# latentnetworks/vimure

Measured on AMD Instinct MI355X. Metric: CAVI iterations/sec (L=4 N=2000 M=200 K=2 synthetic, mutuality on), higher is better.
Workload: dtype f64

## Files before the change

vimure_amd/csrc/sweep_sl.h:

```cpp
#ifndef VMR_SWEEP_SL_H
#define VMR_SWEEP_SL_H

#include "vmr_internal.h"
#include <functional>

#define SL_YM(e) ((e) & 0xfffffu)
#define SL_INR(e) (((e) >> 20) & 1u)
#define SL_X(e) ((e) >> 21)
#define SL_XMAX 2047u
#define SL_YM_ROWS (1u << 20)
#define SL_PF 8
#ifndef SL_PFW
#define SL_PFW 8
#endif
constexpr int sl_pf(int K) { return K <= 2 ? SL_PF : SL_PFW; }
#define SL_SLACK (64 * 64)

struct SlArgs {
  const unsigned* E; const unsigned* rs; const unsigned long long* ebase; const unsigned* perm;
  const unsigned* sy;
  const uint8_t* cls;
  const unsigned* Qt;
  const uint64_t* Rb; const unsigned* rq; const unsigned short* Rm; const unsigned long long* rbase;
  const unsigned* rm2;
  double* rho; const double* logpr;
  const double* par; double* slotR; const double* lutg; double* Hg; double* slotF; double* slotA;
  int Gl;
  int do_hist;
  int yt, hc;
  int sum_a;
  double* nu_acc; double* elbo_dev; int commit_nu;
  int nu_stale;
  unsigned long long* det;
  int lp0;
  int farl;
  double* h0s;
  const unsigned* x0p;
  int lv0r;
  const unsigned* Ez;
  int elbo_cur;
#ifdef SL_DEBUG
  unsigned long long* dbg_t;
#endif
};

struct SlShape { int tpb, yt, hc; size_t smem; };
struct SlUnit { SlArgs a; Geo g; int blk0, nblk; };

#ifndef SL_LIGHT_UPD_K
#define SL_LIGHT_UPD_K 2
#endif
constexpr bool sl_light(int K, bool elbo, bool allfull, bool update) { return !elbo && allfull && (K <= SL_LIGHT_UPD_K || (!update && K <= 4)); }
#ifndef SL_ELBO3_K
#define SL_ELBO3_K 2
#endif
#ifndef SL_ELBO3
#define SL_ELBO3 1
#endif
constexpr int sl_tpb_max(int K, bool elbo, bool allfull, bool update = true) {
  return elbo ? ((SL_ELBO3 && K <= SL_ELBO3_K) ? 768 : (K <= 4 ? 512 : 256)) : (sl_light(K, elbo, allfull, update) ? 1024 : (K <= 3 ? 768 : (K <= 7 ? 512 : 256)));
}
constexpr int sl_tpb_max_b(int K, bool elbo, bool allfull) { return elbo ? sl_tpb_max(K, true, allfull) : (K <= 2 ? 768 : (K <= 7 ? 512 : 256)); }
constexpr int sl_wpe_b(int K, bool elbo, bool allfull) { return elbo ? ((SL_ELBO3 && K <= SL_ELBO3_K) ? 3 : (K <= 4 ? 2 : 1)) : (K <= 2 ? 3 : (K <= 7 ? 2 : 1)); }
// ... 24 lines not shown
```

vimure_amd/csrc/sweep_sl.hip:

```cpp
#include "sweep_sl.h"

#ifndef VMR_K
#error "compile with -DVMR_K=<number of categories>"
#endif
#ifndef SL_WPE
#define SL_WPE sl_wpe(2, false, true)
#endif

template <int K>
struct StepIn {
  double v[K];
  double w[K];
  unsigned cls, qt, tie;
  unsigned x0;
  unsigned e[sl_pf(K)];
};

template <int R> struct RC { static constexpr int value = R; };
template <class V> __device__ __forceinline__ const V* at_bytes(const V* p, unsigned off) {
  return reinterpret_cast<const V*>(reinterpret_cast<const char*>(p) + off);
}
template <class V> __device__ __forceinline__ V* at_bytes(V* p, unsigned off) {
  return reinterpret_cast<V*>(reinterpret_cast<char*>(p) + off);
}
__device__ __forceinline__ double rcp_nr2(double d) {
  double r = __builtin_amdgcn_rcp(d);
  r = fma(fma(-d, r, 1.0), r, r);
  return fma(fma(-d, r, 1.0), r, r);
}
#define SL_INL __attribute__((always_inline))
#ifndef SL_BATCH2
#define SL_BATCH2 8
#endif
template <int K> struct Batch { static constexpr int value = K <= 2 ? SL_BATCH2 : (K <= 4 ? 4 : 2); };

template <int K, bool UPDATE, bool ELBO, bool ALLFULL, bool STORE = true, bool DET = false>
__device__ __forceinline__ void sweep_body(const SlArgs& a, const Geo& g, const unsigned bx, const unsigned gx) {
  extern __shared__ __align__(16) unsigned char smem[];
  constexpr int PFK = sl_pf(K);
  constexpr bool LV0 = !UPDATE && !ELBO && !DET;
  constexpr bool LV0R = UPDATE && K >= 3;
  const int tid = threadIdx.x, lane = tid & 63, nthr = (int)blockDim.x;
  const int wv = __builtin_amdgcn_readfirstlane(tid >> 6), nw = nthr >> 6;
  const int Mp = g.Mp;
  const unsigned ytm = UPDATE ? (unsigned)a.yt * (unsigned)Mp : 0u;
  const unsigned hcm = a.do_hist ? (unsigned)a.hc * (unsigned)Mp : 0u;
  size_t off = 0;
  double* F = reinterpret_cast<double*>(smem + off); off += (size_t)ytm * K * 8;
  const int nHc = (int)hcm * K;
  double* Hc = reinterpret_cast<double*>(smem + off); off += (size_t)nHc * 8;
  double* Gth = reinterpret_cast<double*>(smem + off); off += (size_t)Mp * 8;
  double* Lth = reinterpret_cast<double*>(smem + off); off += UPDATE ? (size_t)Mp * 8 : 0;
  double* As = reinterpret_cast<double*>(smem + off); off += a.sum_a ? (size_t)Mp * K * 8 : 0;
  double* wsum = reinterpret_cast<double*>(smem + off); off += (size_t)g.W * 8;
  double* red = reinterpret_cast<double*>(smem + off); off += 16 * 8;
  double* xt = reinterpret_cast<double*>(smem + off); off += 64 * 8;
  double* lt = reinterpret_cast<double*>(smem + off); off += ELBO ? 256 * 8 : 0;
  double* EthL = reinterpret_cast<double*>(smem + off); off += a.rq ? (size_t)Mp * 8 : 0;
  const ParOff o = par_off(g.L, g.Mp, g.K);
// ... 39 lines not shown
  const double lp0_0 = log(1.0 + eps), lp0_k = log(eps);
  double e_lin = 0.0, e_q = 0.0, e_log = 0.0;
  double accF[K], acc0[K];
#pragma unroll
  for (int k = 0; k < K; ++k) { accF[k] = 0.0; acc0[k] = 0.0; }
  unsigned long long ie_lin = 0ull, ie_q = 0ull, ie_log = 0ull, iaccF[K];
#pragma unroll
  for (int k = 0; k < K; ++k) iaccF[k] = 0ull;
  double* Hl = a.Hg + ((size_t)l * NH + (gb % NH)) * g.Y * Mp * K;
  auto det_H = [&]() SL_INL { return a.det + (size_t)l * g.Y * Mp * K; };
  auto det_A = [&]() SL_INL { return a.det + (size_t)g.L * g.Y * Mp * K + (size_t)l * g.W * 64 * K; };
  auto det_F = [&]() SL_INL { return a.det + (size_t)g.L * g.Y * Mp * K + (size_t)g.L * g.W * 64 * K + (size_t)l * K; };
  auto det_R = [&]() SL_INL { return a.det + (size_t)g.L * g.Y * Mp * K + (size_t)g.L * g.W * 64 * K + (size_t)g.L * K; };
  const unsigned* rsl = a.rs + (size_t)l * (NS + 1);
  const unsigned* syl = a.sy + (size_t)l * NS;
  const unsigned* El = a.E + a.ebase[l];
  const unsigned* pl = (a.rm2 ? a.rm2 : a.perm) + (size_t)l * NS * 64;
  const uint8_t* cl = ALLFULL ? nullptr : a.cls + (size_t)l * T;
  const unsigned* Ql = a.Qt ? a.Qt + (size_t)l * T : nullptr;
  const uint64_t* Rl = a.Rb ? a.Rb + (size_t)l * T * g.W : nullptr;
  double* rl = a.rho + (size_t)l * T * K;
  double* rho_slack = a.rho + (size_t)g.L * T * K;
  const double* lpl = a.logpr + (size_t)l * T * K;
  const unsigned* rql = a.rq ? a.rq + (size_t)l * (T + 1) : nullptr;
  const unsigned short* Rml = a.rq ? a.Rm + a.rbase[l] : nullptr;
  const unsigned lim_y = UPDATE ? (a.do_hist ? (unsigned)min(a.yt, a.hc) : (unsigned)a.yt) : (a.do_hist ? (unsigned)a.hc : 0xffffffffu);
  const unsigned lim1 = (UPDATE && a.yt < g.Y) ? (unsigned)a.yt : 0xffffffffu;
  const unsigned lim2 = (a.do_hist && a.hc < g.Y) ? (unsigned)a.hc : 0xffffffffu;

  const long long Gl_ = a.Gl;
  unsigned* tick = reinterpret_cast<unsigned*>(smem + off); off += 16;
  if (tid == 0) { tick[0] = 2u * (unsigned)nw; tick[1] = 0u; }
  auto step_of = [&](unsigned t) SL_INL -> long long { return (long long)gb + (long long)t * Gl_; };
  auto draw = [&]() SL_INL -> long long {
    unsigned t = 0u;
    if (lane == 0) t = atomicAdd(tick, 1u);
    return step_of((unsigned)__builtin_amdgcn_readfirstlane((int)t));
  };
  long long s = step_of((unsigned)wv), sn = step_of((unsigned)(nw + wv));
  unsigned ea = 0;
  int R = 0;
  unsigned ymax = 0;
  unsigned rgv = 0;
  StepIn<K> P;

  const unsigned lane4 = (unsigned)lane * 4u, laneK8 = (unsigned)lane * (unsigned)(K * 8);
  const unsigned T32 = (unsigned)T;
  auto fetch_range = [&](long long st) SL_INL {
    const unsigned ra = rsl[st + (lane < 1 ? 0 : 1)], ry = syl[st];
    rgv = lane == 2 ? ry : ra;
  };
  auto fetch_tie = [&](StepIn<K>& d, long long st, const bool lp_const = false) SL_INL {
    const size_t row0 = (size_t)st * 64;
    const bool ok = (unsigned)row0 + (unsigned)lane < T32;
    d.qt = 0u; d.tie = 0u;
    if (ALLFULL) d.cls = ok ? 1u : 0u;
    else {
      const unsigned c = (unsigned)*at_bytes(cl + row0, (unsigned)lane);
      d.cls = ok ? c : 0u;
      d.tie = *at_bytes(pl + row0, lane4);
    }
    if (ELBO && Ql) d.qt = *at_bytes(Ql + row0, lane4);
    d.x0 = 0u;
    if (LV0 && a.x0p) d.x0 = *at_bytes(a.x0p + (size_t)l * NS * 64 + row0, lane4);
#pragma unroll
    for (int k = 0; k < K; ++k) { d.v[k] = 0.0; d.w[k] = 0.0; }
    if (UPDATE || ELBO) {
      if (lp_const) {
#pragma unroll
        for (int k = 0; k < K; ++k) d.v[k] = k == 0 ? lp0_0 : lp0_k;
      } else load_k<K>(at_bytes(lpl + row0 * K, laneK8), d.v);
    }
    if (!UPDATE && a.do_hist != 2) load_k<K>(at_bytes(static_cast<const double*>(rl) + row0 * K, laneK8), d.w);
  };
  auto fetch_ent = [&](StepIn<K>& d, unsigned base, auto cntc) SL_INL {
    constexpr int CNT = decltype(cntc)::value;
    const unsigned* pe = El + base;
#pragma unroll
    for (int j = 0; j < CNT; ++j) d.e[j] = *at_bytes(pe + j * 64, lane4);
  };

  if (s < NS) {
    ea = rsl[s];
    R = (int)((rsl[s + 1] - ea) >> 6);
    ymax = syl[s];
    fetch_range(sn < NS ? sn : s);
    fetch_tie(P, s);
    fetch_ent(P, ea, RC<PFK>{});
  }
#ifdef SL_DEBUG
// ... 232 lines not shown
            const double dx = fr[u] ? 0.0 : (double)SL_X(c[u]);
#pragma unroll
            for (int k = 0; k < K; ++k) U[k] = fma(dx, f[u][k], U[k]);
          }
#pragma unroll
          for (int u = 0; u < GB; ++u) {
            if (__any(fr[u])) {
              if (fr[u]) {
                double ff[K];
                f_far(SL_YM(c[u]), ff);
                const double dx = (double)SL_X(c[u]);
#pragma unroll
                for (int k = 0; k < K; ++k) U[k] = fma(dx, ff[k], U[k]);
              }
            }
          }
        }, Rr);
        if (LV0R && a.lv0r && !lv0_off) {
#pragma unroll
          for (int k = 0; k < K; ++k) U[k] += fma(Lla[k], sx1, sl0);
        }
      }
      double aa[K];
#pragma unroll
      for (int k = 0; k < K; ++k) aa[k] = (cur.v[k] + U[k]) - Tt * Ela[k];
      bool done = false;
      if (K == 2) {
        const double d = aa[1] - aa[0];
        const bool safe = fabs(aa[0]) < 700.0 && fabs(aa[1]) < 700.0 && fabs(d) < 700.0;
        if (__all(safe)) {
          const double e = exp_tab(d, xt);
          r[0] = rcp_nr2(1.0 + e);
          r[1] = e * r[0];
          done = true;
        }
      }
      if (!done) {
        double sum = 0.0;
        bool tame = true;
#pragma unroll
        for (int k = 0; k < K; ++k) tame = tame && fabs(aa[k]) < 700.0;
        tame = __all(tame);
        if (tame) {
#pragma unroll
          for (int k = 0; k < K; ++k) r[k] = exp_tab(aa[k], xt);
        } else {
#pragma unroll
          for (int k = 0; k < K; ++k) r[k] = exp(aa[k]);
        }
#pragma unroll
        for (int k = 0; k < K; ++k) sum += r[k];
        if (sum > 0.0) {
#pragma unroll
          for (int k = 0; k < K; ++k) r[k] /= sum;
        }
        if (a.do_hist) {
          double sm = 0.0;
#pragma unroll
// ... 302 lines not shown
    }
  }
  if (ELBO) {
    if (DET) {
      const unsigned long long v1 = wave_isum(ie_lin), v2 = wave_isum(ie_log), v3 = wave_isum(ie_q);
      if (lane == 0) { unsigned long long* dR = det_R(); atomicAdd(&dR[1], v1); atomicAdd(&dR[2], v2); atomicAdd(&dR[3], v3); }
    } else {
      double v1 = block_sum_n(e_lin, red);
      double v2 = block_sum_n(e_log, red);
      double v3 = block_sum_n(e_q, red);
      if (tid == 0) {
        double* out = a.slotR + (size_t)(bx % NSLOT) * 4;
        atomicAdd(&out[1], v1); atomicAdd(&out[2], v2); atomicAdd(&out[3], v3);
      }
    }
  }
#ifdef SL_DEBUG
  if (dbt && lane == 0) dbt[3] = wall_clock64();
#endif
}

#define SL_BOUNDS(K, UPDATE, ELBO, ALLFULL) \
  __launch_bounds__(sl_tpb_max(K, ELBO, ALLFULL, UPDATE), (K == 2 && !ELBO && ALLFULL) ? SL_WPE : sl_wpe(K, ELBO, ALLFULL, UPDATE))
template <int K, bool UPDATE, bool ELBO, bool ALLFULL, bool STORE = true, bool DET = false>
__global__ SL_BOUNDS(K, UPDATE, ELBO, ALLFULL) void k_sweep_sl(SlArgs a, Geo g) {
  sweep_body<K, UPDATE, ELBO, ALLFULL, STORE, DET>(a, g, blockIdx.x, gridDim.x);
}
template <int K, bool UPDATE, bool ELBO, bool ALLFULL, bool STORE = true>
__global__ __launch_bounds__(sl_tpb_max_b(K, ELBO, ALLFULL), sl_wpe_b(K, ELBO, ALLFULL)) void k_sweep_sl_b(const SlUnit* __restrict__ units, const int* __restrict__ blk_unit) {
  const SlUnit& u = units[blk_unit[blockIdx.x]];
  sweep_body<K, UPDATE, ELBO, ALLFULL, STORE>(u.a, u.g, blockIdx.x - (unsigned)u.blk0, (unsigned)u.nblk);
}

template <bool UPDATE, bool ELBO, bool ALLFULL, bool STORE = true, bool DET = false>
static int sl_launch_one(vmr_ctx* h, const SlShape& sh, SlArgs& a) {
  constexpr int K = VMR_K;
  const Geo& g = h->g;
  const long long NS = ((long long)g.N * g.N + 63) / 64, nw = sh.tpb / 64;
  int rc = grid_per_layer(h, k_sweep_sl<K, UPDATE, ELBO, ALLFULL, STORE, DET>, sh.smem, &a.Gl, (NS + nw - 1) / nw, sh.tpb);
  if (rc) return rc;
#ifdef SL_DEBUG
  static unsigned long long* dbg_buf = nullptr;
  const char* tf = h->opt.debug_times[0] ? h->opt.debug_times : nullptr;
  const size_t nwv = (size_t)g.L * a.Gl * nw;
  a.dbg_t = nullptr;
  if (tf) {
    if (!dbg_buf) (void)hipMalloc(&dbg_buf, (size_t)1 << 22);
    if (nwv * 64 <= ((size_t)1 << 22)) a.dbg_t = dbg_buf;
  }
#endif
  hipLaunchKernelGGL((k_sweep_sl<K, UPDATE, ELBO, ALLFULL, STORE, DET>), dim3(g.L * a.Gl), dim3(sh.tpb), sh.smem, h->stream, a, g);
#ifdef SL_DEBUG
  if (a.dbg_t) {
    std::vector<unsigned long long> t(nwv * 8);
    (void)hipStreamSynchronize(h->stream);
    (void)hipMemcpy(t.data(), dbg_buf, nwv * 64, hipMemcpyDeviceToHost);
    if (FILE* f = fopen(tf, "a")) {
      fprintf(f, "launch %d%d hist %d waves %zu tpb %d\n", (int)UPDATE, (int)ELBO, a.do_hist, nwv, sh.tpb);
      for (size_t i = 0; i < nwv; ++i) fprintf(f, "%llu %llu %llu %llu %llu %llu %llu %llu\n", t[i * 8], t[i * 8 + 1], t[i * 8 + 2], t[i * 8 + 3], t[i * 8 + 4], t[i * 8 + 5], t[i * 8 + 6], t[i * 8 + 7]);
      fclose(f);
    }
  }
#endif
  return VMR_OK;
}

#define SL_CAT2(a, b) a##b
#define SL_CAT(a, b) SL_CAT2(a, b)
int SL_CAT(vmr_sl_launch_k, VMR_K)(vmr_ctx* h, int mode, const SlShape& sh, SlArgs& a) {
  if (a.det) {
    if (a.cls == nullptr) {
      switch (mode) {
        case 0: return sl_launch_one<true, false, true, true, true>(h, sh, a);
        case 4: return sl_launch_one<true, false, true, false, true>(h, sh, a);
        case 1: return sl_launch_one<true, true, true, true, true>(h, sh, a);
        case 2: return sl_launch_one<false, true, true, true, true>(h, sh, a);
        default: return sl_launch_one<false, false, true, true, true>(h, sh, a);
      }
    }
    switch (mode) {
      case 0: return sl_launch_one<true, false, false, true, true>(h, sh, a);
      case 4: return sl_launch_one<true, false, false, false, true>(h, sh, a);
      case 1: return sl_launch_one<true, true, false, true, true>(h, sh, a);
      case 2: return sl_launch_one<false, true, false, true, true>(h, sh, a);
      default: return sl_launch_one<false, false, false, true, true>(h, sh, a);
    }
  }
  if (a.cls == nullptr) {
    switch (mode) {
      case 0: return sl_launch_one<true, false, true>(h, sh, a);
      case 1: return sl_launch_one<true, true, true>(h, sh, a);
      case 2: return sl_launch_one<false, true, true>(h, sh, a);
      case 4: return sl_launch_one<true, false, true, false>(h, sh, a);
      default: return sl_launch_one<false, false, true>(h, sh, a);
    }
  }
  switch (mode) {
    case 0: return sl_launch_one<true, false, false>(h, sh, a);
    case 1: return sl_launch_one<true, true, false>(h, sh, a);
    case 2: return sl_launch_one<false, true, false>(h, sh, a);
    case 4: return sl_launch_one<true, false, false, false>(h, sh, a);
    default: return sl_launch_one<false, false, false>(h, sh, a);
  }
}

template <bool UPDATE, bool ELBO, bool ALLFULL, bool STORE = true>
static int sl_launch_batch_one(vmr_ctx* h, hipStream_t st, const SlUnit* units, const int* blk_unit, int nblocks, int tpb, size_t smem) {
  constexpr int K = VMR_K;
  if (smem > 48 * 1024)
    HIPCHK(h, hipFuncSetAttribute(reinterpret_cast<const void*>(k_sweep_sl_b<K, UPDATE, ELBO, ALLFULL, STORE>), hipFuncAttributeMaxDynamicSharedMemorySize, (int)smem));
  hipLaunchKernelGGL((k_sweep_sl_b<K, UPDATE, ELBO, ALLFULL, STORE>), dim3(nblocks), dim3(tpb), smem, st, units, blk_unit);
  return VMR_OK;
}
int SL_CAT(vmr_sl_launch_batch_k, VMR_K)(vmr_ctx* h, hipStream_t st, int mode, int allfull, const SlUnit* units, const int* blk_unit, int nblocks,
                                          int tpb, size_t smem) {
  if (mode == 3) return allfull ? sl_launch_batch_one<false, false, true>(h, st, units, blk_unit, nblocks, tpb, smem)
                                : sl_launch_batch_one<false, false, false>(h, st, units, blk_unit, nblocks, tpb, smem);
  if (mode == 4) return allfull ? sl_launch_batch_one<true, false, true, false>(h, st, units, blk_unit, nblocks, tpb, smem)
                                : sl_launch_batch_one<true, false, false, false>(h, st, units, blk_unit, nblocks, tpb, smem);
  if (allfull) return mode ? sl_launch_batch_one<true, true, true>(h, st, units, blk_unit, nblocks, tpb, smem)
                           : sl_launch_batch_one<true, false, true>(h, st, units, blk_unit, nblocks, tpb, smem);
  return mode ? sl_launch_batch_one<true, true, false>(h, st, units, blk_unit, nblocks, tpb, smem)
              : sl_launch_batch_one<true, false, false>(h, st, units, blk_unit, nblocks, tpb, smem);
}
```

vimure_amd/csrc/vimure_hip.hip:

```cpp
#include "vmr_internal.h"
#include "sweep_sl.h"
#include "sweep_gen.h"

thread_local std::string g_create_err;



template <int SH>
__device__ __forceinline__ unsigned nz_flags16(uint4 v) {
  const unsigned M = 0x7f7f7f7fu;
  unsigned t0 = ((v.x & M) + M) | v.x, t1 = ((v.y & M) + M) | v.y;
  unsigned t2 = ((v.z & M) + M) | v.z, t3 = ((v.w & M) + M) | v.w;
  unsigned f = (t0 >> (7 - SH)) & (0x01010101u << SH);
  f |= (t1 >> (6 - SH)) & (0x02020202u << SH);
  f |= (t2 >> (5 - SH)) & (0x04040404u << SH);
  f |= (t3 >> (4 - SH)) & (0x08080808u << SH);
  return f;
}
__device__ __forceinline__ void flag_pos(int bit, int& chunk, int& byte) {
  const int lo = bit & 31;
  chunk = ((bit >> 5) << 1) | ((lo >> 2) & 1);
  byte = ((lo & 3) << 2) | (lo >> 3);
}

// ... 332 lines not shown
                           size_t n, double eps) {
  for (size_t q = blockIdx.x * (size_t)blockDim.x + threadIdx.x; q < n; q += (size_t)gridDim.x * blockDim.x) {
    double v = pr[q];
    rho[q] = v;
    logpr[q] = log(v + eps);
  }
}

__global__ void k_init_rho_pos(const double* __restrict__ pr, double* __restrict__ rho, double* __restrict__ logpr,
                               const unsigned* __restrict__ perm, size_t T, size_t NS, int L, int K, double eps,
                               const unsigned* __restrict__ rs, int* __restrict__ not_onehot) {
  const size_t n = (size_t)L * T * K;
  bool bad = false;
  for (size_t q = blockIdx.x * (size_t)blockDim.x + threadIdx.x; q < n; q += (size_t)gridDim.x * blockDim.x) {
    const size_t row = q / K, k = q - row * K, l = row / T, pos = row - l * T;
    const double v = pr[(l * T + perm[l * NS * 64 + pos]) * K + k];
    rho[q] = v;
    logpr[q] = log(v + eps);
    const unsigned* rsl = rs + l * (NS + 1);
    const size_t st = pos >> 6;
    if (rsl[st + 1] == rsl[st] && v != (k == 0 ? 1.0 : 0.0)) bad = true;
  }
  if (bad) atomicOr(not_onehot, 1);
}

__global__ void k_build_lut(const double* __restrict__ par, double* __restrict__ lutg, Geo g) {
  const ParOff o = par_off(g.L, g.Mp, g.K);
  const int l = blockIdx.x;
  const double* Eth = par + o.E_th + (size_t)l * g.Mp;
  for (int q = threadIdx.x; q < g.W * 256; q += blockDim.x) {
    int n = q >> 4, e = q & 15;
    double v = 0.0;
    for (int u = 0; u < 4; ++u) {
      int m = n * 4 + u;
      if (((e >> u) & 1) && m < g.Mp) v += Eth[m];
    }
    lutg[(size_t)l * g.W * 256 + q] = v;
  }
}

__global__ void k_derive_all(double* par, Geo g) {
  ParOff o = par_off(g.L, g.Mp, g.K);
  int tid = blockIdx.x * blockDim.x + threadIdx.x, nth = gridDim.x * blockDim.x;
  for (int q = tid; q < g.L * g.Mp; q += nth) {
    int m = q % g.Mp;
    if (m < g.M) {
// ... 1173 lines not shown
  return (size_t)g.nt * g.stride + (size_t)g.nt * g.K * 8 + shmem_hc(g) + shmem_q() + 16;
}
static size_t shmem_rho(const Geo& g, bool update, bool elbo) {
  size_t n = (size_t)g.nt * g.stride + (size_t)g.nt * g.W * 8 + (size_t)g.W * 8 + (size_t)g.Mp * 8 + 64 + shmem_ct(g) +
             2 * (size_t)g.nt * g.K * 8 + shmem_q();
  if (update && !g.two_pass) n += shmem_hc(g);
  if (elbo) n += (size_t)g.Mp * 8 + (size_t)g.nt * 4;
  return n + 16;
}

#define SP_LDS_MAX (160 * 1024)

static SlShape sl_shape(const vmr_ctx* h, bool update, bool elbo, bool hist) {
  const Geo& g = h->g;
  SlShape s{std::max(64, std::min((update || elbo) ? h->sp_tpb : h->st_tpb, sl_tpb_max(g.K, elbo, h->all_full != 0, update)) & ~63), update ? g.yt : 0, hist ? g.hc : 0, 0};
  auto bytes = [&]() { return sl_smem(g, s.yt, s.hc, update, elbo, hist); };
  while (bytes() > SP_LDS_MAX && (s.yt > 0 || s.hc > 0)) { if (s.yt >= s.hc && s.yt > 0) --s.yt; else --s.hc; }
  s.smem = bytes();
  return s;
}
static SlArgs sl_args(const vmr_ctx* h, const SlShape& sh, int do_hist, int sum_a = 0) {
  return SlArgs{h->E, h->rs, h->ebase, h->perm, h->sy, h->cls_p, h->Qt_p, h->Rb, h->rq, h->Rm, h->rbase, h->rm2, h->rho, h->logpr, h->par, h->slotR,
                h->lutg, h->Hg, h->slotF, h->slotA, 1, do_hist, sh.yt, sh.hc, sum_a, nullptr, nullptr, 0, 0, nullptr, h->lp0 ? 1 : 0, h->g.farl, (do_hist == 1 && h->g.two_pass && sh.hc >= 1) ? h->h0s : nullptr, (do_hist == 1 && h->g.two_pass && sh.hc >= 1 && h->h0s) ? h->x0p : nullptr,
                (h->h0s && h->g.two_pass && !h->opt.no_lv0r) ? 1 : 0, h->E + h->n_slots, 0};
}
static int sl_launch(vmr_ctx* h, int mode, const SlShape& sh, SlArgs& a) {
  sl_launch_fn fn = vmr_sl_launcher(h->g.K);
  if (!fn) return fail(h, VMR_EINVAL, "this build of libvimure_hip.so holds no sweep kernel for this K");
  return fn(h, mode, sh, a);
}

#ifdef VMR_DEV
#define DISPATCH_K(K_, ...)                         \
  switch (K_) {                                     \
    case 2: { constexpr int KK = 2; __VA_ARGS__; } break; \
    default: break;                                 \
  }
#else
#define DISPATCH_K(K_, ...)                         \
  switch (K_) {                                     \
    case 2: { constexpr int KK = 2; __VA_ARGS__; } break; \
    case 3: { constexpr int KK = 3; __VA_ARGS__; } break; \
    case 4: { constexpr int KK = 4; __VA_ARGS__; } break; \
    case 5: { constexpr int KK = 5; __VA_ARGS__; } break; \
    case 6: { constexpr int KK = 6; __VA_ARGS__; } break; \
    case 7: { constexpr int KK = 7; __VA_ARGS__; } break; \
    case 8: { constexpr int KK = 8; __VA_ARGS__; } break; \
// ... 509 lines not shown

static void read_opts(VmrOpts& o) {
  memset(&o, 0, sizeof o);
  auto set = [](const char* n) { return getenv(n) != nullptr; };
  auto num = [](const char* n, int dflt) { const char* e = getenv(n); return e ? atoi(e) : dflt; };
  if (const char* f = getenv("VMR_FORMAT")) o.format = !strcmp(f, "dense") ? 1 : !strcmp(f, "sparse") ? 2 : 0;
  o.deterministic = num("VMR_DETERMINISTIC", 0) != 0;
  o.graph = num("VMR_GRAPH", 0) != 0;
  o.debug = num("VMR_DEBUG", 0);
  o.levels = num("VMR_LEVELS", 64);
  o.two_pass = num("VMR_TWO_PASS", 0);
  o.farl = num("VMR_FARL", 0);
  o.yt = set("VMR_YT") ? std::max(0, num("VMR_YT", 0)) : -1;
  o.hc = set("VMR_HC") ? std::max(0, num("VMR_HC", 0)) : -1;
  o.tpb = num("VMR_TPB", 0);
  o.st_tpb = num("VMR_ST_TPB", 0);
  o.no_level0 = set("VMR_NO_LEVEL0");
  o.no_x0 = set("VMR_NO_X0");
  o.no_lv0r = set("VMR_NO_LV0R");
  o.no_level_sort = set("VMR_NO_LEVEL_SORT");
  o.no_rlists = set("VMR_NO_RLISTS");
  o.no_rm2 = set("VMR_NO_RM2");
  o.no_lp0 = set("VMR_NO_LP0");
  o.always_store_rho = set("VMR_ALWAYS_STORE_RHO");
  o.debug_lazy_rho = set("VMR_DEBUG_LAZY_RHO");
  o.gen_hsum = num("VMR_GEN_HSUM", 0);
  o.gen_no_lds_h = set("VMR_GEN_NO_LDS_H");
  o.gen_dbg = num("VMR_GEN_DBG", 0);
  o.batch_fg = set("VMR_BATCH_FG") ? std::max(1, std::min(FG_G, num("VMR_BATCH_FG", 0))) : 0;
  if (const char* t = getenv("VMR_DEBUG_TIMES")) snprintf(o.debug_times, sizeof o.debug_times, "%s", t);
}

static int create_ctx(vmr_ctx** out, hipDeviceProp_t* prop, int device, int L, int N, int M, int K, int mutuality, double eps, bool lists_only = false) {
  if (L < 1 || N < 1 || M < 1) return fail(nullptr, VMR_EINVAL, "L, N, M must be positive");
  if (K < 2 || K > KGEN_MAX) return fail(nullptr, VMR_EINVAL, "K must be in [2, 256]");
  int ndev = 0;
  CK(hipGetDeviceCount(&ndev));
  if (device < 0 || device >= ndev) return fail(nullptr, VMR_EINVAL, "no such HIP device");
  CK(hipSetDevice(device));
  CK(hipGetDeviceProperties(prop, device));
  vmr_ctx* h = new vmr_ctx();
  *out = h;
  h->device = device;
  Geo& g = h->g;
  g.L = L; g.N = N; g.M = M; g.K = K; g.mut = mutuality ? 1 : 0; g.eps = eps;
  g.gen = K > KMAX ? 1 : 0; g.wide = 0;
// ... 826 lines not shown
  if (M > 65535) return fail(nullptr, VMR_EINVAL, "M exceeds 65535 (M_COO_MAX): the mask lists hold 16-bit reporter indices");
  int mb = 13;
  while ((1 << mb) < (M + 15) / 16 * 16) ++mb;
  if ((((unsigned __int128)L * (unsigned)N * (unsigned)N) << mb) >> 64)
    return fail(nullptr, VMR_EINVAL, "L * N^2 * 2^ceil(log2 M) must stay below 2^64 (the 64-bit sort keys of the coordinates)");
  vmr_ctx* h = nullptr;
  hipDeviceProp_t prop;
  int rc = create_ctx(&h, &prop, device, L, N, M, K, mutuality, eps, true);
  if (!rc) h->coo_mb = mb;
  if (!rc) rc = create_coo(h, prop, nx, xl, xi, xj, xm, xv, nr, rl, ri, rj, rm, data_on_device);
  if (rc) { if (h) vmr_destroy(h); return rc; }
  *out = h;
  return VMR_OK;
}

extern "C" {

void vmr_destroy(vmr_handle h) {
  if (!h) return;
  (void)hipSetDevice(h->device);
  if (h->stream) (void)hipStreamSynchronize(h->stream);
  for (auto& e : h->evs) { (void)hipEventDestroy(e.a); (void)hipEventDestroy(e.b); }
  for (auto& e : h->graphs) (void)hipGraphExecDestroy(e.ex);
  void* ptrs[] = {h->drw, h->x0p, h->h0s, h->far_pos, h->far_ent, h->far_base, h->EX, h->gen_s1, h->rm2, h->det_buf, h->fr_slots, h->nu_acc, h->fin_g, h->perm, h->sy, h->cls_p, h->Qt_p, h->nat, h->rho_snap, h->par_snap, h->rq, h->Rm, h->rbase, h->E, h->rs, h->Cg, h->Qt, h->ebase, h->rcls, h->X, h->Rb, h->cov, h->sumx, h->rho, h->logpr, h->par, h->slotA, h->slotR, h->elbo_dev, h->lutg, h->Hg, h->xmax, h->slotF, h->npartial};
  for (void* p : ptrs) if (p) (void)hipFree(p);
  if (h->stream2) { (void)hipStreamSynchronize(h->stream2); (void)hipStreamDestroy(h->stream2); }
  if (h->ev_fork) (void)hipEventDestroy(h->ev_fork);
  if (h->ev_join) (void)hipEventDestroy(h->ev_join);
  if (h->stream) (void)hipStreamDestroy(h->stream);
  delete h;
}

int vmr_data_stats(vmr_handle h, double* sum_x, uint8_t* coverage) {
  if (!h) return VMR_EINVAL;
  HIPCHK(h, hipSetDevice(h->device));
  unsigned long long v = 0;
  if (sum_x) HIPCHK(h, hipMemcpyAsync(&v, h->sumx, 8, hipMemcpyDeviceToHost, h->stream));
  if (coverage) HIPCHK(h, hipMemcpyAsync(coverage, h->cov, (size_t)h->g.L * h->g.N * h->g.N, hipMemcpyDeviceToHost, h->stream));
  HIPCHK(h, hipStreamSynchronize(h->stream));
  if (sum_x) *sum_x = (double)v;
  return VMR_OK;
}

static int upload_lm(vmr_ctx* h, size_t off, const double* src, double pad) {
  const Geo& g = h->g;
  std::vector<double> buf((size_t)g.L * g.Mp, pad);
  for (int l = 0; l < g.L; ++l) memcpy(&buf[(size_t)l * g.Mp], src + (size_t)l * g.M, (size_t)g.M * 8);
// ... 40 lines not shown
  if ((rc = upload_lm(h, o.g_shp, gamma_shp, 1.0))) return rc;
  if ((rc = upload_lm(h, o.g_rte, gamma_rte, 1.0))) return rc;
  if ((rc = h2d(h, h->par + o.p_shp, phi_shp, (size_t)g.L * g.K * 8))) return rc;
  if ((rc = h2d(h, h->par + o.p_rte, phi_rte, (size_t)g.L * g.K * 8))) return rc;
  double nu[2] = {nu_shp, nu_rte};
  if ((rc = h2d(h, h->par + o.sc + SC_NU_SHP, nu, 16))) return rc;
  const size_t n = (size_t)g.L * g.N * g.N * g.K;
  const double* src = pr_rho;
  if (h->perm) {
    if (!pr_rho_on_device) {
      if (!h->nat) HIPCHK(h, hipMalloc(&h->nat, n * 8));
      HIPCHK(h, hipMemcpyAsync(h->nat, pr_rho, n * 8, hipMemcpyHostToDevice, h->stream));
      src = h->nat;
    }
    const size_t T_ = (size_t)g.N * g.N;
    int* flag = reinterpret_cast<int*>(h->elbo_dev + 7);
    HIPCHK(h, hipMemsetAsync(flag, 0, 4, h->stream));
    hipLaunchKernelGGL(k_init_rho_pos, dim3(4096), dim3(256), 0, h->stream, src, h->rho, h->logpr, h->perm, T_, (T_ + 63) / 64, g.L, g.K, g.eps,
                       h->rs, flag);
    int nf = 1;
    HIPCHK(h, hipMemcpyAsync(&nf, flag, 4, hipMemcpyDeviceToHost, h->stream));
    HIPCHK(h, hipStreamSynchronize(h->stream));
    h->lp0 = nf == 0 && !h->opt.no_lp0;
  } else {
    if (!pr_rho_on_device) {
      HIPCHK(h, hipMemcpyAsync(h->logpr, pr_rho, n * 8, hipMemcpyHostToDevice, h->stream));
      src = h->logpr;
    }
    hipLaunchKernelGGL(k_init_rho, dim3(4096), dim3(256), 0, h->stream, src, h->rho, h->logpr, n, g.eps);
  }
  HIPCHK(h, hipGetLastError());
  hipLaunchKernelGGL(k_derive_all, dim3(8), dim3(256), 0, h->stream, h->par, g);
  HIPCHK(h, hipGetLastError());
  hipLaunchKernelGGL(k_build_lut, dim3(g.L), dim3(256), 0, h->stream, h->par, h->lutg, g);
  HIPCHK(h, hipGetLastError());
  HIPCHK(h, hipMemsetAsync(h->slotF, 0, (size_t)g.L * NSLOT * g.K * 8, h->stream));
  HIPCHK(h, hipStreamSynchronize(h->stream));
  drop_graphs(h);
  h->have_state = true;
  h->restored = false;
  h->rho_stale = false;
  h->h_valid = false;
  h->f_valid = false;
  h->a_valid = false;
  h->h_zero = false; h->a_zero = false;
  if (h->h0s) HIPCHK(h, hipMemsetAsync(h->h0s, 0, (size_t)h->g.L * NSLOT * h->g.K * 8, h->stream));
// ... 679 lines not shown
  if (lists) *lists = h->rq ? 1 : 0;
  if (listed) *listed = h->n_rm;
  return VMR_OK;
}

int vmr_sweep_shape(vmr_handle h, int* passes, int* lds_levels, uint64_t* far_reports) {
  if (!h) return VMR_EINVAL;
  if (passes) *passes = h->g.two_pass ? 2 : 1;
  if (lds_levels) *lds_levels = h->g.gen ? 0 : h->g.hc;
  if (far_reports) *far_reports = (h->g.farl && !h->far_off.empty()) ? h->far_off.back() : 0ull;
  return VMR_OK;
}

int vmr_kernel_bytes(vmr_handle h, int kernel_class, double* bytes) {
  if (!h || !bytes) return VMR_EINVAL;
  const Geo& g = h->g;
  const double V = (double)g.L * g.N * g.N * g.M;
  const double SX = V, SR = V / 8.0, Srho = 8.0 * g.L * (double)g.N * g.N * g.K;
  if (h->sparse) {
    const double ties = (double)g.L * g.N * g.N;
    const double E = (g.wide ? 8.0 : 4.0) * (double)h->nnz, RP = 4.0 * (ties / 64.0 + g.L);
    const double mask = h->all_full ? 0.0 : ties + (h->rq ? 4.0 * ties + 2.0 * (double)h->n_rm : (double)h->n_partial * g.W * 8.0);
    const double Q = g.mut ? 4.0 * ties : 0.0;
    switch (kernel_class) {
      case VMR_KERNEL_GAMMA_MASK: *bytes = ties + (h->rq ? 4.0 * ties + 2.0 * (double)h->n_rm : (double)h->n_partial * g.W * 8.0) + Srho; break;
      case VMR_KERNEL_GAMMA_COUNTS:
        *bytes = ((h->x0p && g.two_pass) ? 4.0 * (double)h->stat_slots + 4.0 * ties : E) + RP + Srho;
        break;
      case VMR_KERNEL_RHO: *bytes = E + RP + mask + 2.0 * Srho; break;
      case VMR_KERNEL_RHO_NOSTORE: *bytes = E + RP + mask + Srho; break;
      case VMR_KERNEL_ELBO: *bytes = E + RP + mask + Q + 2.0 * Srho; break;
      case VMR_KERNEL_RHO_ELBO: *bytes = E + RP + mask + Q + 2.0 * Srho; break;
      default: *bytes = 0.0; break;
    }
    return VMR_OK;
  }
  switch (kernel_class) {
    case VMR_KERNEL_GAMMA_MASK: *bytes = SR + Srho; break;
    case VMR_KERNEL_GAMMA_COUNTS: *bytes = SX + Srho; break;
    case VMR_KERNEL_PHI: *bytes = 0.0; break;
    case VMR_KERNEL_RHO: *bytes = SX + SR + 2.0 * Srho; break;
    case VMR_KERNEL_ELBO: *bytes = SX + SR + 2.0 * Srho; break;
    case VMR_KERNEL_RHO_ELBO: *bytes = SX + SR + 2.0 * Srho; break;
    default: *bytes = 0.0; break;
  }
  return VMR_OK;
}

}
```

vimure_amd/csrc/vmr_internal.h:

```cpp
#ifndef VMR_INTERNAL_H
#define VMR_INTERNAL_H
#include <hip/hip_runtime.h>
#include <hipcub/hipcub.hpp>
#include <stdint.h>
#include <stdio.h>
#include <string.h>
#include <math.h>
#include <stdlib.h>
#include <string>
#include <vector>
#include <utility>
#include <algorithm>
#include <chrono>
#include <type_traits>

#include "vimure_hip.h"

#define VMR_VERSION "vimure_hip 0.1 (gfx950)"
#define TPB 256
#ifndef VMR_LB_COUNTS
#define VMR_LB_COUNTS 4
#endif
#ifndef VMR_LB_RHO
#define VMR_LB_RHO 3
// ... 28 lines not shown
  double eps;
  int det;
  int det_sh;
  int det_shr;
  int gen;
  int farl;
  int wide;
  int det_sha;
};
#define DET_SH_A 30
#define DET_SH2 30
__device__ __forceinline__ unsigned long long det_fx(double v, int sh) { return (unsigned long long)__double2ll_rn(ldexp(v, sh)); }
__device__ __forceinline__ double det_back(unsigned long long u, int sh) { return ldexp((double)(long long)u, -sh); }

#define NSLOT 8

struct VmrOpts {
  int format;
  bool deterministic, graph;
  int debug, levels;
  int two_pass, farl;
  int yt, hc;
  int tpb, st_tpb;
  bool no_level0, no_x0, no_lv0r, no_level_sort, no_rlists, no_rm2, no_lp0;
  bool always_store_rho, debug_lazy_rho;
  int gen_hsum;
  bool gen_no_lds_h;
  int gen_dbg;
  int batch_fg;
  char debug_times[256];
};

struct vmr_ctx {
  Geo g;
  VmrOpts opt;
  int device;
  hipStream_t stream;
  hipStream_t stream2 = nullptr;
  hipEvent_t ev_fork = nullptr, ev_join = nullptr;
  std::string err;
  uint8_t* X = nullptr;
  uint64_t* Rb = nullptr;
  uint8_t* cov = nullptr;
  void* drw = nullptr;
  size_t drw_cap = 0;
  uint8_t* rcls = nullptr;
  int sparse = 0;
// ... 11 lines not shown
  int all_full = 0;
  unsigned* perm = nullptr;
  unsigned* sy = nullptr;
  unsigned* far_pos = nullptr;
  unsigned* far_ent = nullptr;
  unsigned long long* far_base = nullptr;
  std::vector<unsigned long long> far_off;
  double* h0s = nullptr;
  unsigned long long stat_slots = 0;
  unsigned* x0p = nullptr;
  bool elbo_split = false;
  uint8_t* cls_p = nullptr;
  unsigned* Qt_p = nullptr;
  double* nat = nullptr;
  unsigned* rq = nullptr;
  unsigned short* Rm = nullptr;
  unsigned long long* rbase = nullptr;
  unsigned long long n_rm = 0;
  unsigned rm_maxrow = 0;
  unsigned* rm2 = nullptr;
  int coo_mb = 13;
  unsigned long long* sumx = nullptr;
  double *rho = nullptr, *logpr = nullptr;
  double* par = nullptr;
  struct GraphEntry { int n; bool lazy_last; unsigned sig0, sig1; hipGraphExec_t ex; };
  std::vector<GraphEntry> graphs;
  bool use_graphs = false;
  unsigned long long* det_buf = nullptr;
  double* fr_slots = nullptr;
  double *rho_snap = nullptr, *par_snap = nullptr;
  bool have_snap = false;
  bool lp0 = false;
  bool rho_stale = false;
  bool restored = false;
  size_t par_doubles = 0;
  double *slotA = nullptr, *slotR = nullptr;
  double* Hg = nullptr;
  bool h_valid = false;
  double* slotF = nullptr;
  bool f_valid = false;
  bool a_valid = false;
  bool a_zero = true;
  bool h_reduced = false;
  bool h_zero = false;
  bool fin_attr = false, ml_attr = false;
  unsigned long long* npartial = nullptr;
// ... 268 lines not shown
```

Before: 5657.

## Precompute K=2 log-prior difference to halve logpr reads in rho update sweep

For K=2, a one-time kernel computes the per-tie difference logpr[1]-logpr[0] and the per-layer max absolute log-prior. The update sweep then loads one double per tie instead of two. The overflow check uses the precomputed bounds and only reloads full logpr when the check fails. This adds a new template variant and a small setup kernel, and changes the order of floating-point additions slightly.

```diff
diff --git a/vimure_amd/csrc/sweep_sl.h b/vimure_amd/csrc/sweep_sl.h
--- a/vimure_amd/csrc/sweep_sl.h
+++ b/vimure_amd/csrc/sweep_sl.h
@@ -39,6 +39,7 @@
   int lv0r;
   const unsigned* Ez;
   int elbo_cur;
+  const double* lpd; const double* lpb;
 #ifdef SL_DEBUG
   unsigned long long* dbg_t;
 #endif
diff --git a/vimure_amd/csrc/sweep_sl.hip b/vimure_amd/csrc/sweep_sl.hip
--- a/vimure_amd/csrc/sweep_sl.hip
+++ b/vimure_amd/csrc/sweep_sl.hip
@@ -34,7 +34,7 @@
 #endif
 template <int K> struct Batch { static constexpr int value = K <= 2 ? SL_BATCH2 : (K <= 4 ? 4 : 2); };
 
-template <int K, bool UPDATE, bool ELBO, bool ALLFULL, bool STORE = true, bool DET = false>
+template <int K, bool UPDATE, bool ELBO, bool ALLFULL, bool STORE = true, bool DET = false, bool LPD = false>
 __device__ __forceinline__ void sweep_body(const SlArgs& a, const Geo& g, const unsigned bx, const unsigned gx) {
   extern __shared__ __align__(16) unsigned char smem[];
   constexpr int PFK = sl_pf(K);
@@ -120,6 +120,9 @@
   double* rl = a.rho + (size_t)l * T * K;
   double* rho_slack = a.rho + (size_t)g.L * T * K;
   const double* lpl = a.logpr + (size_t)l * T * K;
+  constexpr bool LPDV = LPD && K == 2 && UPDATE && !ELBO;
+  const double* lpdl = LPDV ? a.lpd + (size_t)l * T : nullptr;
+  const double lpb0 = (K == 2 && UPDATE) ? a.lpb[2 * l] : 0.0, lpb1 = (K == 2 && UPDATE) ? a.lpb[2 * l + 1] : 0.0;
   const unsigned* rql = a.rq ? a.rq + (size_t)l * (T + 1) : nullptr;
   const unsigned short* Rml = a.rq ? a.Rm + a.rbase[l] : nullptr;
   const unsigned lim_y = UPDATE ? (a.do_hist ? (unsigned)min(a.yt, a.hc) : (unsigned)a.yt) : (a.do_hist ? (unsigned)a.hc : 0xffffffffu);
@@ -163,7 +166,10 @@
     if (LV0 && a.x0p) d.x0 = *at_bytes(a.x0p + (size_t)l * NS * 64 + row0, lane4);
 #pragma unroll
     for (int k = 0; k < K; ++k) { d.v[k] = 0.0; d.w[k] = 0.0; }
-    if (UPDATE || ELBO) {
+    if (LPDV) {
+      if (lp_const) d.v[0] = lp0_k - lp0_0;
+      else d.v[0] = *at_bytes(lpdl + row0, (unsigned)lane * 8u);
+    } else if (UPDATE || ELBO) {
       if (lp_const) {
 #pragma unroll
         for (int k = 0; k < K; ++k) d.v[k] = k == 0 ? lp0_0 : lp0_k;
@@ -442,18 +448,31 @@
         }
       }
       double aa[K];
-#pragma unroll
-      for (int k = 0; k < K; ++k) aa[k] = (cur.v[k] + U[k]) - Tt * Ela[k];
       bool done = false;
       if (K == 2) {
-        const double d = aa[1] - aa[0];
-        const bool safe = fabs(aa[0]) < 700.0 && fabs(aa[1]) < 700.0 && fabs(d) < 700.0;
+        double c[K];
+#pragma unroll
+        for (int k = 0; k < K; ++k) c[k] = fma(-Tt, Ela[k], U[k]);
+        const double d = ((LPDV ? cur.v[0] : cur.v[K - 1] - cur.v[0]) + c[K - 1]) - c[0];
+        bool safe = fabs(c[0]) + lpb0 < 700.0 && fabs(c[K - 1]) + lpb1 < 700.0 && fabs(d) < 700.0;
+        if (!__all(safe)) {
+          double v[K];
+#pragma unroll
+          for (int k = 0; k < K; ++k) v[k] = cur.v[k];
+          if (LPDV) load_k<K>(at_bytes(lpl + row0 * K, laneK8), v);
+#pragma unroll
+          for (int k = 0; k < K; ++k) aa[k] = v[k] + c[k];
+          safe = fabs(aa[0]) < 700.0 && fabs(aa[K - 1]) < 700.0 && fabs(d) < 700.0;
+        }
         if (__all(safe)) {
           const double e = exp_tab(d, xt);
           r[0] = rcp_nr2(1.0 + e);
-          r[1] = e * r[0];
+          r[K - 1] = e * r[0];
           done = true;
         }
+      } else {
+#pragma unroll
+        for (int k = 0; k < K; ++k) aa[k] = (cur.v[k] + U[k]) - Tt * Ela[k];
       }
       if (!done) {
         double sum = 0.0;
@@ -802,22 +821,22 @@
 
 #define SL_BOUNDS(K, UPDATE, ELBO, ALLFULL) \
   __launch_bounds__(sl_tpb_max(K, ELBO, ALLFULL, UPDATE), (K == 2 && !ELBO && ALLFULL) ? SL_WPE : sl_wpe(K, ELBO, ALLFULL, UPDATE))
-template <int K, bool UPDATE, bool ELBO, bool ALLFULL, bool STORE = true, bool DET = false>
+template <int K, bool UPDATE, bool ELBO, bool ALLFULL, bool STORE = true, bool DET = false, bool LPD = false>
 __global__ SL_BOUNDS(K, UPDATE, ELBO, ALLFULL) void k_sweep_sl(SlArgs a, Geo g) {
-  sweep_body<K, UPDATE, ELBO, ALLFULL, STORE, DET>(a, g, blockIdx.x, gridDim.x);
-}
-template <int K, bool UPDATE, bool ELBO, bool ALLFULL, bool STORE = true>
+  sweep_body<K, UPDATE, ELBO, ALLFULL, STORE, DET, LPD>(a, g, blockIdx.x, gridDim.x);
+}
+template <int K, bool UPDATE, bool ELBO, bool ALLFULL, bool STORE = true, bool LPD = false>
 __global__ __launch_bounds__(sl_tpb_max_b(K, ELBO, ALLFULL), sl_wpe_b(K, ELBO, ALLFULL)) void k_sweep_sl_b(const SlUnit* __restrict__ units, const int* __restrict__ blk_unit) {
   const SlUnit& u = units[blk_unit[blockIdx.x]];
-  sweep_body<K, UPDATE, ELBO, ALLFULL, STORE>(u.a, u.g, blockIdx.x - (unsigned)u.blk0, (unsigned)u.nblk);
-}
-
-template <bool UPDATE, bool ELBO, bool ALLFULL, bool STORE = true, bool DET = false>
-static int sl_launch_one(vmr_ctx* h, const SlShape& sh, SlArgs& a) {
+  sweep_body<K, UPDATE, ELBO, ALLFULL, STORE, false, LPD>(u.a, u.g, blockIdx.x - (unsigned)u.blk0, (unsigned)u.nblk);
+}
+
+template <bool UPDATE, bool ELBO, bool ALLFULL, bool STORE = true, bool DET = false, bool LPD = false>
+static int sl_launch_one_(vmr_ctx* h, const SlShape& sh, SlArgs& a) {
   constexpr int K = VMR_K;
   const Geo& g = h->g;
   const long long NS = ((long long)g.N * g.N + 63) / 64, nw = sh.tpb / 64;
-  int rc = grid_per_layer(h, k_sweep_sl<K, UPDATE, ELBO, ALLFULL, STORE, DET>, sh.smem, &a.Gl, (NS + nw - 1) / nw, sh.tpb);
+  int rc = grid_per_layer(h, k_sweep_sl<K, UPDATE, ELBO, ALLFULL, STORE, DET, LPD>, sh.smem, &a.Gl, (NS + nw - 1) / nw, sh.tpb);
   if (rc) return rc;
 #ifdef SL_DEBUG
   static unsigned long long* dbg_buf = nullptr;
@@ -829,7 +848,7 @@
     if (nwv * 64 <= ((size_t)1 << 22)) a.dbg_t = dbg_buf;
   }
 #endif
-  hipLaunchKernelGGL((k_sweep_sl<K, UPDATE, ELBO, ALLFULL, STORE, DET>), dim3(g.L * a.Gl), dim3(sh.tpb), sh.smem, h->stream, a, g);
+  hipLaunchKernelGGL((k_sweep_sl<K, UPDATE, ELBO, ALLFULL, STORE, DET, LPD>), dim3(g.L * a.Gl), dim3(sh.tpb), sh.smem, h->stream, a, g);
 #ifdef SL_DEBUG
   if (a.dbg_t) {
     std::vector<unsigned long long> t(nwv * 8);
@@ -843,6 +862,12 @@
   }
 #endif
   return VMR_OK;
+}
+
+template <bool UPDATE, bool ELBO, bool ALLFULL, bool STORE = true, bool DET = false>
+static int sl_launch_one(vmr_ctx* h, const SlShape& sh, SlArgs& a) {
+  if (VMR_K == 2 && UPDATE && !ELBO && a.lpd) return sl_launch_one_<UPDATE, ELBO, ALLFULL, STORE, DET, VMR_K == 2 && UPDATE && !ELBO>(h, sh, a);
+  return sl_launch_one_<UPDATE, ELBO, ALLFULL, STORE, DET>(h, sh, a);
 }
 
 #define SL_CAT2(a, b) a##b
@@ -884,22 +909,28 @@
   }
 }
 
-template <bool UPDATE, bool ELBO, bool ALLFULL, bool STORE = true>
-static int sl_launch_batch_one(vmr_ctx* h, hipStream_t st, const SlUnit* units, const int* blk_unit, int nblocks, int tpb, size_t smem) {
+template <bool UPDATE, bool ELBO, bool ALLFULL, bool STORE = true, bool LPD = false>
+static int sl_launch_batch_one_(vmr_ctx* h, hipStream_t st, const SlUnit* units, const int* blk_unit, int nblocks, int tpb, size_t smem) {
   constexpr int K = VMR_K;
   if (smem > 48 * 1024)
-    HIPCHK(h, hipFuncSetAttribute(reinterpret_cast<const void*>(k_sweep_sl_b<K, UPDATE, ELBO, ALLFULL, STORE>), hipFuncAttributeMaxDynamicSharedMemorySize, (int)smem));
-  hipLaunchKernelGGL((k_sweep_sl_b<K, UPDATE, ELBO, ALLFULL, STORE>), dim3(nblocks), dim3(tpb), smem, st, units, blk_unit);
+    HIPCHK(h, hipFuncSetAttribute(reinterpret_cast<const void*>(k_sweep_sl_b<K, UPDATE, ELBO, ALLFULL, STORE, LPD>), hipFuncAttributeMaxDynamicSharedMemorySize, (int)smem));
+  hipLaunchKernelGGL((k_sweep_sl_b<K, UPDATE, ELBO, ALLFULL, STORE, LPD>), dim3(nblocks), dim3(tpb), smem, st, units, blk_unit);
   return VMR_OK;
+}
+template <bool UPDATE, bool ELBO, bool ALLFULL, bool STORE = true>
+static int sl_launch_batch_one(vmr_ctx* h, hipStream_t st, bool lpd, const SlUnit* units, const int* blk_unit, int nblocks, int tpb, size_t smem) {
+  if (VMR_K == 2 && UPDATE && !ELBO && lpd) return sl_launch_batch_one_<UPDATE, ELBO, ALLFULL, STORE, VMR_K == 2 && UPDATE && !ELBO>(h, st, units, blk_unit, nblocks, tpb, smem);
+  return sl_launch_batch_one_<UPDATE, ELBO, ALLFULL, STORE>(h, st, units, blk_unit, nblocks, tpb, smem);
 }
 int SL_CAT(vmr_sl_launch_batch_k, VMR_K)(vmr_ctx* h, hipStream_t st, int mode, int allfull, const SlUnit* units, const int* blk_unit, int nblocks,
                                           int tpb, size_t smem) {
-  if (mode == 3) return allfull ? sl_launch_batch_one<false, false, true>(h, st, units, blk_unit, nblocks, tpb, smem)
-                                : sl_launch_batch_one<false, false, false>(h, st, units, blk_unit, nblocks, tpb, smem);
-  if (mode == 4) return allfull ? sl_launch_batch_one<true, false, true, false>(h, st, units, blk_unit, nblocks, tpb, smem)
-                                : sl_launch_batch_one<true, false, false, false>(h, st, units, blk_unit, nblocks, tpb, smem);
-  if (allfull) return mode ? sl_launch_batch_one<true, true, true>(h, st, units, blk_unit, nblocks, tpb, smem)
-                           : sl_launch_batch_one<true, false, true>(h, st, units, blk_unit, nblocks, tpb, smem);
-  return mode ? sl_launch_batch_one<true, true, false>(h, st, units, blk_unit, nblocks, tpb, smem)
-              : sl_launch_batch_one<true, false, false>(h, st, units, blk_unit, nblocks, tpb, smem);
-}
+  const bool lpd = h->lpd != nullptr;
+  if (mode == 3) return allfull ? sl_launch_batch_one<false, false, true>(h, st, lpd, units, blk_unit, nblocks, tpb, smem)
+                                : sl_launch_batch_one<false, false, false>(h, st, lpd, units, blk_unit, nblocks, tpb, smem);
+  if (mode == 4) return allfull ? sl_launch_batch_one<true, false, true, false>(h, st, lpd, units, blk_unit, nblocks, tpb, smem)
+                                : sl_launch_batch_one<true, false, false, false>(h, st, lpd, units, blk_unit, nblocks, tpb, smem);
+  if (allfull) return mode ? sl_launch_batch_one<true, true, true>(h, st, lpd, units, blk_unit, nblocks, tpb, smem)
+                           : sl_launch_batch_one<true, false, true>(h, st, lpd, units, blk_unit, nblocks, tpb, smem);
+  return mode ? sl_launch_batch_one<true, true, false>(h, st, lpd, units, blk_unit, nblocks, tpb, smem)
+              : sl_launch_batch_one<true, false, false>(h, st, lpd, units, blk_unit, nblocks, tpb, smem);
+}
diff --git a/vimure_amd/csrc/vimure_hip.hip b/vimure_amd/csrc/vimure_hip.hip
--- a/vimure_amd/csrc/vimure_hip.hip
+++ b/vimure_amd/csrc/vimure_hip.hip
@@ -378,6 +378,25 @@
     if (rsl[st + 1] == rsl[st] && v != (k == 0 ? 1.0 : 0.0)) bad = true;
   }
   if (bad) atomicOr(not_onehot, 1);
+}
+
+__global__ __launch_bounds__(256) void k_lpd(const double* __restrict__ logpr, double* __restrict__ lpd, unsigned long long* __restrict__ lpb, size_t T, int L) {
+  for (int l = 0; l < L; ++l) {
+    unsigned long long m0 = 0ull, m1 = 0ull;
+    for (size_t q = blockIdx.x * (size_t)blockDim.x + threadIdx.x; q < T; q += (size_t)gridDim.x * blockDim.x) {
+      const size_t row = (size_t)l * T + q;
+      const double v0 = logpr[row * 2], v1 = logpr[row * 2 + 1];
+      if (lpd) lpd[row] = v1 - v0;
+      m0 = max(m0, (unsigned long long)__double_as_longlong(fabs(v0)));
+      m1 = max(m1, (unsigned long long)__double_as_longlong(fabs(v1)));
+    }
+#pragma unroll
+    for (int o2 = 32; o2 > 0; o2 >>= 1) {
+      m0 = max(m0, (unsigned long long)__shfl_xor((long long)m0, o2, 64));
+      m1 = max(m1, (unsigned long long)__shfl_xor((long long)m1, o2, 64));
+    }
+    if ((threadIdx.x & 63) == 0) { atomicMax(&lpb[2 * l], m0); atomicMax(&lpb[2 * l + 1], m1); }
+  }
 }
 
 __global__ void k_build_lut(const double* __restrict__ par, double* __restrict__ lutg, Geo g) {
@@ -1597,7 +1616,7 @@
 static SlArgs sl_args(const vmr_ctx* h, const SlShape& sh, int do_hist, int sum_a = 0) {
   return SlArgs{h->E, h->rs, h->ebase, h->perm, h->sy, h->cls_p, h->Qt_p, h->Rb, h->rq, h->Rm, h->rbase, h->rm2, h->rho, h->logpr, h->par, h->slotR,
                 h->lutg, h->Hg, h->slotF, h->slotA, 1, do_hist, sh.yt, sh.hc, sum_a, nullptr, nullptr, 0, 0, nullptr, h->lp0 ? 1 : 0, h->g.farl, (do_hist == 1 && h->g.two_pass && sh.hc >= 1) ? h->h0s : nullptr, (do_hist == 1 && h->g.two_pass && sh.hc >= 1 && h->h0s) ? h->x0p : nullptr,
-                (h->h0s && h->g.two_pass && !h->opt.no_lv0r) ? 1 : 0, h->E + h->n_slots, 0};
+                (h->h0s && h->g.two_pass && !h->opt.no_lv0r) ? 1 : 0, h->E + h->n_slots, 0, h->lpd, h->lpb};
 }
 static int sl_launch(vmr_ctx* h, int mode, const SlShape& sh, SlArgs& a) {
   sl_launch_fn fn = vmr_sl_launcher(h->g.K);
@@ -2153,6 +2172,7 @@
   o.no_rlists = set("VMR_NO_RLISTS");
   o.no_rm2 = set("VMR_NO_RM2");
   o.no_lp0 = set("VMR_NO_LP0");
+  o.no_lpd = set("VMR_NO_LPD");
   o.always_store_rho = set("VMR_ALWAYS_STORE_RHO");
   o.debug_lazy_rho = set("VMR_DEBUG_LAZY_RHO");
   o.gen_hsum = num("VMR_GEN_HSUM", 0);
@@ -3025,7 +3045,7 @@
   if (h->stream) (void)hipStreamSynchronize(h->stream);
   for (auto& e : h->evs) { (void)hipEventDestroy(e.a); (void)hipEventDestroy(e.b); }
   for (auto& e : h->graphs) (void)hipGraphExecDestroy(e.ex);
-  void* ptrs[] = {h->drw, h->x0p, h->h0s, h->far_pos, h->far_ent, h->far_base, h->EX, h->gen_s1, h->rm2, h->det_buf, h->fr_slots, h->nu_acc, h->fin_g, h->perm, h->sy, h->cls_p, h->Qt_p, h->nat, h->rho_snap, h->par_snap, h->rq, h->Rm, h->rbase, h->E, h->rs, h->Cg, h->Qt, h->ebase, h->rcls, h->X, h->Rb, h->cov, h->sumx, h->rho, h->logpr, h->par, h->slotA, h->slotR, h->elbo_dev, h->lutg, h->Hg, h->xmax, h->slotF, h->npartial};
+  void* ptrs[] = {h->drw, h->x0p, h->h0s, h->far_pos, h->far_ent, h->far_base, h->EX, h->gen_s1, h->rm2, h->det_buf, h->fr_slots, h->nu_acc, h->fin_g, h->perm, h->sy, h->cls_p, h->Qt_p, h->nat, h->rho_snap, h->par_snap, h->rq, h->Rm, h->rbase, h->E, h->rs, h->Cg, h->Qt, h->ebase, h->rcls, h->X, h->Rb, h->cov, h->sumx, h->rho, h->logpr, h->lpd, h->lpb, h->par, h->slotA, h->slotR, h->elbo_dev, h->lutg, h->Hg, h->xmax, h->slotF, h->npartial};
   for (void* p : ptrs) if (p) (void)hipFree(p);
   if (h->stream2) { (void)hipStreamSynchronize(h->stream2); (void)hipStreamDestroy(h->stream2); }
   if (h->ev_fork) (void)hipEventDestroy(h->ev_fork);
@@ -3112,6 +3132,16 @@
     HIPCHK(h, hipMemcpyAsync(&nf, flag, 4, hipMemcpyDeviceToHost, h->stream));
     HIPCHK(h, hipStreamSynchronize(h->stream));
     h->lp0 = nf == 0 && !h->opt.no_lp0;
+    if (g.K == 2 && !g.gen) {
+      if (!h->lpb) HIPCHK(h, hipMalloc(&h->lpb, (size_t)g.L * 2 * 8));
+      if (!h->lpd && !h->opt.no_lpd) {
+        HIPCHK(h, hipMalloc(&h->lpd, ((size_t)g.L * T_ + 64) * 8));
+        HIPCHK(h, hipMemsetAsync(h->lpd + (size_t)g.L * T_, 0, (size_t)64 * 8, h->stream));
+      }
+      HIPCHK(h, hipMemsetAsync(h->lpb, 0, (size_t)g.L * 2 * 8, h->stream));
+      hipLaunchKernelGGL(k_lpd, dim3(1024), dim3(256), 0, h->stream, h->logpr, h->lpd, reinterpret_cast<unsigned long long*>(h->lpb), T_, g.L);
+      HIPCHK(h, hipGetLastError());
+    }
   } else {
     if (!pr_rho_on_device) {
       HIPCHK(h, hipMemcpyAsync(h->logpr, pr_rho, n * 8, hipMemcpyHostToDevice, h->stream));
@@ -3837,13 +3867,14 @@
     const double E = (g.wide ? 8.0 : 4.0) * (double)h->nnz, RP = 4.0 * (ties / 64.0 + g.L);
     const double mask = h->all_full ? 0.0 : ties + (h->rq ? 4.0 * ties + 2.0 * (double)h->n_rm : (double)h->n_partial * g.W * 8.0);
     const double Q = g.mut ? 4.0 * ties : 0.0;
+    const double Slp = h->lpd ? 8.0 * ties : Srho;
     switch (kernel_class) {
       case VMR_KERNEL_GAMMA_MASK: *bytes = ties + (h->rq ? 4.0 * ties + 2.0 * (double)h->n_rm : (double)h->n_partial * g.W * 8.0) + Srho; break;
       case VMR_KERNEL_GAMMA_COUNTS:
         *bytes = ((h->x0p && g.two_pass) ? 4.0 * (double)h->stat_slots + 4.0 * ties : E) + RP + Srho;
         break;
-      case VMR_KERNEL_RHO: *bytes = E + RP + mask + 2.0 * Srho; break;
-      case VMR_KERNEL_RHO_NOSTORE: *bytes = E + RP + mask + Srho; break;
+      case VMR_KERNEL_RHO: *bytes = E + RP + mask + Slp + Srho; break;
+      case VMR_KERNEL_RHO_NOSTORE: *bytes = E + RP + mask + Slp; break;
       case VMR_KERNEL_ELBO: *bytes = E + RP + mask + Q + 2.0 * Srho; break;
       case VMR_KERNEL_RHO_ELBO: *bytes = E + RP + mask + Q + 2.0 * Srho; break;
       default: *bytes = 0.0; break;
diff --git a/vimure_amd/csrc/vmr_internal.h b/vimure_amd/csrc/vmr_internal.h
--- a/vimure_amd/csrc/vmr_internal.h
+++ b/vimure_amd/csrc/vmr_internal.h
@@ -74,7 +74,7 @@
   int two_pass, farl;
   int yt, hc;
   int tpb, st_tpb;
-  bool no_level0, no_x0, no_lv0r, no_level_sort, no_rlists, no_rm2, no_lp0;
+  bool no_level0, no_x0, no_lv0r, no_level_sort, no_rlists, no_rm2, no_lp0, no_lpd;
   bool always_store_rho, debug_lazy_rho;
   int gen_hsum;
   bool gen_no_lds_h;
@@ -132,6 +132,7 @@
   int coo_mb = 13;
   unsigned long long* sumx = nullptr;
   double *rho = nullptr, *logpr = nullptr;
+  double *lpd = nullptr, *lpb = nullptr;
   double* par = nullptr;
   struct GraphEntry { int n; bool lazy_last; unsigned sig0, sig1; hipGraphExec_t ex; };
   std::vector<GraphEntry> graphs;
```

Result: faster. 6008 (median of 6 runs) (+6.2%).
